# tnwei/waternet

Hardware: NVIDIA H100
Metric: images/sec at 1080p batch16 (preprocess + gated-fusion forward, uint8 in -> uint8 out) (higher is better)
Workload: dtype bf16 + fp8 corrections (v = hi + lo: hi x hi in bf16, both correction terms of the heavy layers as one e4m3 MMA; fp32 accumulate; 3-term bf16 elsewhere)

## Files before the change

### waternet_b200/csrc/conv_umma.cu

```cuda
#include "umma_conv.cuh"

namespace wn {

__device__ __forceinline__ bool pack_pixel(const PackInArgs& a, int n, int y, int x, float* v) {
  bool exact = true;
#pragma unroll
  for (int t = 0; t < 4; t++)
#pragma unroll
    for (int c = 0; c < 3; c++) {
      float f = __fmul_rn(a.p[t][n * a.s[t][0] + c * a.s[t][1] + y * a.s[t][2] + x * a.s[t][3]], 255.0f);
      float r = rintf(f);
      if (fabsf(f - r) <= 6.103515625e-5f && r >= 0.f && r <= 255.f) f = r; else exact = false;
      v[t * 3 + c] = f;
    }
  return exact;
}
template <bool HI>
__device__ __forceinline__ void store_packed(uint4* o, int hw, float* v) {
  v[12] = v[13] = v[14] = v[15] = 0.f;
  uint32_t hi[8], lo[8];
#pragma unroll
  for (int j = 0; j < 16; j += 2) {
    if constexpr (HI) {
      const __nv_bfloat162 hb = __floats2bfloat162_rn(v[j], v[j + 1]);
      hi[j >> 1] = *reinterpret_cast<const uint32_t*>(&hb);
      lo[j >> 1] = 0u;
    } else {
      split_bf16x2(v[j], v[j + 1], hi[j >> 1], lo[j >> 1]);
    }
  }
  o[0] = make_uint4(hi[0], hi[1], hi[2], hi[3]);
  o[hw] = make_uint4(hi[4], hi[5], hi[6], hi[7]);
  o[2 * (size_t)hw] = make_uint4(lo[0], lo[1], lo[2], lo[3]);
  o[3 * (size_t)hw] = make_uint4(lo[4], lo[5], lo[6], lo[7]);
}
__device__ __forceinline__ bool pack_slot_pixel(const PackInArgs& a, const SlotPixel& p, float* v) {
  return pack_pixel(a, p.img, p.y, p.x, v);
}
__device__ __forceinline__ bool pack_slot_pixel(const PackInArgs* __restrict__ imgs, const SlotPixel& p, float* v) {
  return pack_pixel(imgs[p.img], 0, p.y, p.x, v);
}

template <class Geom, class In, bool PLANES, bool FLAG, bool HI = false>
__global__ void __launch_bounds__(256)
pack_inputs_kernel(Geom geo, In in, uint4* __restrict__ out, int* __restrict__ exact_flag) {
  const int pix = blockIdx.x * 256 + threadIdx.x;
  const int hw = geo.slot_hw();
  bool exact = true;
  if (pix < hw) {
    const SlotPixel p = geo.at(blockIdx.y, pix);
    float v[16];
#pragma unroll
    for (int j = 0; j < 12; j++) v[j] = 0.f;
    if (p.valid) exact = pack_slot_pixel(in, p, v);
    if constexpr (PLANES) store_packed<HI>(out + (size_t)blockIdx.y * 4 * hw + pix, hw, v);
  }
  if constexpr (FLAG)
    if (!__syncthreads_and(exact) && threadIdx.x == 0) atomicExch(exact_flag, 0);
}

template <bool PLANES, bool FLAG, class Geom, class In>
static int launch_pack(wn_handle* h, const Geom& geo, const In& in, int count, uint4* act0, int* flag, bool reset,
                       cudaStream_t stream, bool hi = false) {
  TimedScope ts(h, kSlotPack, stream);
  if (reset) WN_CUDA(cudaMemsetAsync(flag, 1, sizeof(int), stream));
  const dim3 grid((unsigned)(((size_t)geo.slot_hw() + 255) / 256), count);
  if (PLANES && hi)
    pack_inputs_kernel<Geom, In, PLANES, FLAG, true><<<grid, 256, 0, stream>>>(geo, in, act0, flag);
  else
    pack_inputs_kernel<Geom, In, PLANES, FLAG><<<grid, 256, 0, stream>>>(geo, in, act0, flag);
  WN_LAUNCH_CHECK(h);
  return WN_OK;
}
int pack_inputs(wn_handle* h, const GridGeom& geo, const PackInArgs& in, int count, uint4* act0, int* flag,
                cudaStream_t stream, bool hi) {
  if (!act0) return launch_pack<false, true>(h, geo, in, count, nullptr, flag, true, stream);
  if (flag) return launch_pack<true, true>(h, geo, in, count, act0, flag, true, stream, hi);
  return launch_pack<true, false>(h, geo, in, count, act0, nullptr, false, stream, hi);
}
int pack_inputs(wn_handle* h, const TableGeom& geo, const PackInArgs* imgs, int count, uint4* act0, int* flag,
                cudaStream_t stream, bool hi) {
  if (!act0) return launch_pack<false, true>(h, geo, imgs, count, nullptr, flag, false, stream);
  return launch_pack<true, false>(h, geo, imgs, count, act0, nullptr, false, stream, hi);
}

__global__ void __launch_bounds__(256) store_kept_kernel(const float* __restrict__ src, int cs, int c0, int c,
                                                         float* __restrict__ dst, GridGeom geo) {
  const int pix = blockIdx.x * 256 + threadIdx.x;
  const int hw = geo.slot_hw();
  if (pix >= hw) return;
  const SlotPixel p = geo.at(blockIdx.y, pix);
  if (!p.kept) return;
  const float* s = src + ((size_t)blockIdx.y * cs + c0) * hw + pix;
  float* d = dst + (size_t)p.img * c * p.ihw + p.o;
  for (int k = 0; k < c; k++) d[k * p.ihw] = s[(size_t)k * hw];
}

enum UmmaLayer {
  kL1 = 0,
  kC2, kC3, kC4, kC5, kC6, kC7,
  kC8,
  kR2,
  kR3,
  kRL1,
  kNumUmmaLayers
};
struct UmmaLayerSpec {
  int ks, cinpad, npad, epi, concat, nblk, tps, slot;
  bool f8;
  int mw, ng, wgs;
};
static constexpr UmmaLayerSpec kSpecs[kNumUmmaLayers] = {
    {7, 16, 224, kEpiAct, 0, 1, 1, 0, false, 1, 1, 2},
    {5, 128, 128, kEpiAct, 0, 1, 5, 1, true, 1, 1, 2},
    {3, 128, 128, kEpiAct, 0, 1, 3, 2, true, 1, 1, 3},
    {1, 128, 64, kEpiAct, 1, 1, 1, 3, false, 1, 1, 3},
    {7, 64, 64, kEpiAct, 1, 1, 7, 4, true, 2, 1, 2},
    {5, 64, 64, kEpiAct, 1, 1, 5, 5, true, 2, 1, 2},
    {3, 64, 64, kEpiAct, 1, 1, 9, 6, true, 2, 1, 2},
    {3, 64, 16, kEpiSigmoid, 1, 1, 9, 7, false, 1, 1, 3},
    {5, 96, 32, kEpiAct, 1, 3, 5, 9, true, 1, 1, 3},
    {3, 96, 16, kEpiGate, 1, 1, 9, 10, false, 1, 1, 3},
    {7, 16, 96, kEpiAct, 0, 1, 1, 8, false, 1, 1, 3}};
#ifdef WN_UMMA_WGS2
static constexpr int layer_wgs(int) { return 2; }
#else
static constexpr int layer_wgs(int li) { return kSpecs[li].wgs; }
#endif

static_assert(kSpecs[kC2].f8 == kSpecs[kR2].f8, "L1 writes one format for both of its consumers");
static constexpr bool writes_f8(int li) { return li < kR3 && li != kC8 && kSpecs[li + 1].f8; }

static __global__ void __launch_bounds__(256)
mirror_u8_kernel(const uint8_t* __restrict__ src, PeerOut peers, size_t bytes, const int* __restrict__ run_if) {
  if (run_if && *run_if == 0) return;
  const size_t stride = (size_t)gridDim.x * blockDim.x, i0 = (size_t)blockIdx.x * blockDim.x + threadIdx.x;
#pragma unroll
  for (int k = 0; k < WN_MAX_PEERS; k++) {
    if (k >= peers.n) continue;
    uint8_t* dst = peers.p[k];
    const size_t vecs = (((reinterpret_cast<uintptr_t>(src) | reinterpret_cast<uintptr_t>(dst)) & 15) == 0) ? bytes / 16 : 0;
    for (size_t i = i0; i < vecs; i += stride) reinterpret_cast<uint4*>(dst)[i] = reinterpret_cast<const uint4*>(src)[i];
    for (size_t i = vecs * 16 + i0; i < bytes; i += stride) dst[i] = src[i];
  }
}
int mirror_u8(wn_handle* h, const uint8_t* src, const PeerOut& peers, size_t bytes, const int* run_if, cudaStream_t stream) {
  if (peers.n <= 0 || bytes == 0) return WN_OK;
  mirror_u8_kernel<<<4 * h->sm_count, 256, 0, stream>>>(src, peers, bytes, run_if);
  WN_LAUNCH_CHECK(h);
  return WN_OK;
}

struct UmmaWeights {
  uint8_t* stages8[kNumUmmaLayers];
  float* scale8[kNumUmmaLayers];
  int* overflow_dev;
  int* overflow_host;
  uint8_t* stages[kNumUmmaLayers];
  float* bias[kNumUmmaLayers];
  float* dense;
};

static size_t stage_bytes_total(const UmmaLayerSpec& s) { return (size_t)(s.cinpad / 16) * s.ks * s.ks * s.npad * 64; }

int umma_pack_weights(wn_handle* h, const float* const* params, cudaStream_t stream) {
  if (!h->umma) h->umma = (UmmaWeights*)calloc(1, sizeof(UmmaWeights));
  for (int i = 0; i < kNumUmmaLayers; i++) {
    if (!h->umma->stages[i]) WN_CUDA(cudaMalloc(&h->umma->stages[i], stage_bytes_total(kSpecs[i])));
    if (!h->umma->bias[i]) WN_CUDA(cudaMalloc(&h->umma->bias[i], kSpecs[i].npad * kSpecs[i].nblk * sizeof(float)));
    if (kSpecs[i].f8) {
      if (!h->umma->stages8[i]) WN_CUDA(cudaMalloc(&h->umma->stages8[i], stage_bytes_total(kSpecs[i])));
      if (!h->umma->scale8[i]) WN_CUDA(cudaMalloc(&h->umma->scale8[i], 4 * sizeof(float)));
    }
  }
  if (!h->umma->dense) WN_CUDA(cudaMalloc(&h->umma->dense, (size_t)224 * 128 * 49 * sizeof(float)));
  if (!h->umma->overflow_dev) WN_CUDA(cudaMalloc(&h->umma->overflow_dev, sizeof(int)));
  if (!h->umma->overflow_host) WN_CUDA(cudaHostAlloc(&h->umma->overflow_host, sizeof(int), cudaHostAllocDefault));
  UmmaWeights* u = h->umma;
  *u->overflow_host = 0;
  WN_CUDA(cudaMemsetAsync(u->overflow_dev, 0, sizeof(int), stream));
  auto W = [&](int conv) { return params[2 * conv]; };
  auto B = [&](int conv) { return params[2 * conv + 1]; };
  for (int li = 0; li < kNumUmmaLayers; li++) {
    const UmmaLayerSpec& s = kSpecs[li];
    const int kk = s.ks * s.ks;
    const int rows = s.npad * s.nblk;
    WN_CUDA(cudaMemsetAsync(u->dense, 0, (size_t)rows * s.cinpad * kk * sizeof(float), stream));
    WN_CUDA(cudaMemsetAsync(u->bias[li], 0, rows * sizeof(float), stream));
    auto scatter = [&](int conv, int co, int ci, int row_off, int split, int base0, int base1) -> int {
      scatter_weights_kernel<<<128, 256, 0, stream>>>(W(conv), u->dense, co, ci, kk, s.cinpad, row_off, split,
                                                      base0, base1, li == kL1 || li == kRL1 ? 255.0f : 1.0f);
      WN_LAUNCH_CHECK(h);
      scatter_bias_kernel<<<1, 256, 0, stream>>>(B(conv), u->bias[li], co, row_off);
      WN_LAUNCH_CHECK(h);
      return WN_OK;
    };
    int rc = WN_OK;
    if (li == kL1) {
      rc = scatter(0, 128, 12, 0, 12, 0, 0);
      for (int r = 0; r < 3 && !rc; r++)
        rc = scatter(8 + 3 * r, 32, 6, 128 + 32 * r, 3, 0, 3 * (r + 1));
    } else if (li >= kC2 && li <= kC8) {
      const int conv = li;
      const LayerDesc& d = kCmg[conv];
      rc = scatter(conv, d.cout, d.cin, 0, d.cin, 0, 0);
    } else if (li == kR2) {
      for (int r = 0; r < 3 && !rc; r++) rc = scatter(8 + 3 * r + 1, 32, 32, 32 * r, 32, 32 * r, 0);
    } else if (li == kRL1) {
      for (int r = 0; r < 3 && !rc; r++) rc = scatter(8 + 3 * r, 32, 6, 32 * r, 3, 0, 3 * (r + 1));
    } else {
      for (int r = 0; r < 3 && !rc; r++) rc = scatter(8 + 3 * r + 2, 3, 32, 3 * r, 32, 32 * r, 0);
    }
    if (rc) return rc;
    const int gw = s.npad / s.ng;
    const size_t group_bytes = stage_bytes_total(s) / s.ng;
    for (int g = 0; g < s.ng; g++) {
      pack_stages_kernel<<<256, 256, 0, stream>>>(u->dense, (__nv_bfloat16*)(u->stages[li] + g * group_bytes), gw,
                                                  s.cinpad, kk, s.concat, s.nblk, g * gw);
      WN_LAUNCH_CHECK(h);
    }
    if (s.f8) {
      WN_CUDA(cudaMemsetAsync(u->scale8[li], 0, 4 * sizeof(float), stream));
      f8_absmax_kernel<<<64, 256, 0, stream>>>(u->dense, (size_t)rows * s.cinpad * kk, u->scale8[li]);
      WN_LAUNCH_CHECK(h);
      f8_scale_finish_kernel<<<1, 1, 0, stream>>>(u->scale8[li]);
      WN_LAUNCH_CHECK(h);
      for (int g = 0; g < s.ng; g++) {
        pack_stages_f8_kernel<<<256, 256, 0, stream>>>(u->dense, u->stages8[li] + g * group_bytes, u->scale8[li], gw,
                                                       s.cinpad, kk, s.nblk, g * gw);
        WN_LAUNCH_CHECK(h);
      }
    }
  }
  return WN_OK;
}

void umma_free(wn_handle* h) {
  if (!h->umma) return;
  for (int i = 0; i < kNumUmmaLayers; i++) {
    if (h->umma->stages[i]) cudaFree(h->umma->stages[i]);
    if (h->umma->bias[i]) cudaFree(h->umma->bias[i]);
    if (h->umma->stages8[i]) cudaFree(h->umma->stages8[i]);
    if (h->umma->scale8[i]) cudaFree(h->umma->scale8[i]);
  }
  if (h->umma->dense) cudaFree(h->umma->dense);
  if (h->umma->overflow_dev) cudaFree(h->umma->overflow_dev);
  if (h->umma->overflow_host) cudaFreeHost(h->umma->overflow_host);
  free(h->umma);
  h->umma = nullptr;
}

static constexpr size_t kUmmaBytesPerPixel = 64 + 512 + 512 + 384 + 384 + 12;

static constexpr long long kDefaultChunkPixels = 8ll << 20;
static int umma_chunk(long long cap, int n, int h, int w) {
  if (cap <= 0 || cap > kDefaultChunkPixels) cap = kDefaultChunkPixels;
  long long per = (long long)h * w;
  long long nb = cap / (per > 0 ? per : 1);
  if (nb < 1) nb = 1;
  return nb < n ? (int)nb : n;
}
int umma_chunk_images(const wn_handle* h, int n, int height, int width) {
  return umma_chunk(h ? h->chunk_pixels : 0, n, height, width);
}

size_t umma_forward_workspace_bytes(int n, int h, int w) {
  const size_t nb = (size_t)umma_chunk(0, n, h, w);
  return nb * h * w * kUmmaBytesPerPixel + nb * h * 64 + 4096;
}

// ... 579 lines not shown
```

### waternet_b200/csrc/umma_conv.cuh

```cuda
#pragma once

#include <cuda.h>
#include <cuda_bf16.h>

#include "common.cuh"
#include "wgmma_ops.cuh"

namespace wn {

__device__ __forceinline__ uint32_t smem_u32(const void* p) {
  return (uint32_t)__cvta_generic_to_shared(p);
}
__device__ __forceinline__ void mbar_init(uint64_t* bar, uint32_t count) {
  asm volatile("mbarrier.init.shared::cta.b64 [%0], %1;" ::"r"(smem_u32(bar)), "r"(count));
}
__device__ __forceinline__ void mbar_wait(uint64_t* bar, uint32_t parity) {
  for (uint32_t it = 0; it < (1u << 26); it++) {
    uint32_t done;
    asm volatile(
        "{\n\t.reg .pred p;\n\t"
        "mbarrier.try_wait.parity.shared::cta.b64 p, [%1], %2;\n\t"
        "selp.u32 %0, 1, 0, p;\n\t}"
        : "=r"(done)
        : "r"(smem_u32(bar)), "r"(parity)
        : "memory");
    if (done) return;
  }
  __trap();
}
__device__ __forceinline__ void mbar_arrive(uint64_t* bar) {
  asm volatile("mbarrier.arrive.shared::cta.b64 _, [%0];" ::"r"(smem_u32(bar)) : "memory");
}
__device__ __forceinline__ void mbar_expect_tx(uint64_t* bar, uint32_t bytes) {
  asm volatile("mbarrier.arrive.expect_tx.shared::cta.b64 _, [%0], %1;" ::"r"(smem_u32(bar)), "r"(bytes)
               : "memory");
}
__device__ __forceinline__ void tma_load_5d(void* dst, const CUtensorMap* tmap, uint64_t* bar, int c0,
                                            int c1, int c2, int c3, int c4) {
  asm volatile(
      "cp.async.bulk.tensor.5d.shared::cluster.global.mbarrier::complete_tx::bytes [%0], [%1, {%3, %4, %5, %6, %7}], [%2];"
      ::"r"(smem_u32(dst)), "l"(tmap), "r"(smem_u32(bar)), "r"(c0), "r"(c1), "r"(c2), "r"(c3), "r"(c4)
      : "memory");
}
__device__ __forceinline__ void bulk_load(void* dst, const void* src, uint32_t bytes, uint64_t* bar) {
  asm volatile(
      "cp.async.bulk.shared::cluster.global.mbarrier::complete_tx::bytes [%0], [%1], %2, [%3];" ::"r"(
          smem_u32(dst)),
      "l"(src), "r"(bytes), "r"(smem_u32(bar))
      : "memory");
}
__device__ __forceinline__ uint64_t make_desc(uint32_t addr, uint32_t lbo, uint32_t sbo) {
  return (uint64_t)((addr >> 4) & 0x3fff) | ((uint64_t)((lbo >> 4) & 0x3fff) << 16) |
         ((uint64_t)((sbo >> 4) & 0x3fff) << 32);
}
__device__ __forceinline__ void wg_fence() { asm volatile("wgmma.fence.sync.aligned;" ::: "memory"); }
__device__ __forceinline__ void wg_commit() { asm volatile("wgmma.commit_group.sync.aligned;" ::: "memory"); }
template <int PENDING>
__device__ __forceinline__ void wg_wait() { asm volatile("wgmma.wait_group.sync.aligned %0;" ::"n"(PENDING) : "memory"); }
__device__ __forceinline__ void wg_bar(int id) { asm volatile("bar.sync %0, 128;" ::"r"(id) : "memory"); }
__device__ __forceinline__ uint32_t pack_e4m3x4(float f0, float f1, float f2, float f3) {
  uint16_t lo, hi;
  asm("cvt.rn.satfinite.e4m3x2.f32 %0, %1, %2;" : "=h"(lo) : "f"(f1), "f"(f0));
  asm("cvt.rn.satfinite.e4m3x2.f32 %0, %1, %2;" : "=h"(hi) : "f"(f3), "f"(f2));
  return (uint32_t)lo | ((uint32_t)hi << 16);
}
__device__ __forceinline__ uint16_t pack_e4m3x2(float f0, float f1) {
  uint16_t v;
  asm("cvt.rn.satfinite.e4m3x2.f32 %0, %1, %2;" : "=h"(v) : "f"(f1), "f"(f0));
  return v;
}

enum Epilogue { kEpiAct = 0, kEpiSigmoid = 1, kEpiGate = 2, kEpiDgrad = 3 };

constexpr int kStageLd = 36;

constexpr int kFmtIn8 = 1, kFmtOut8 = 2, kFmtHi = 4;
constexpr int kWgs3ProducerRegs = 24, kWgs3ConsumerRegs = 160;
template <int KS, int CIN_PAD, int NPAD, int CONCAT = 0, int NBLK = 1, int TPS = 1, int FMT = 0, int MW = 1,
          int NG = 1, int WGS = 2>
struct UmmaCfg {
  static constexpr bool F8IN = (FMT & kFmtIn8) != 0;
  static constexpr bool HI = (FMT & kFmtHi) != 0;
  static constexpr bool DUAL = CONCAT != 0 && !HI;
  static constexpr int TILE_W = 8 * MW, TILE_H = 8 * WGS;
  static constexpr int CONSUMER_WARPS = 4 * WGS;
  static constexpr int WARP_A = CONSUMER_WARPS, WARP_B = CONSUMER_WARPS + 1;
  static constexpr int THREADS = WGS == 2 ? 320 : 512;
  static constexpr int HALO_W = TILE_W + KS - 1, HALO_H = TILE_H + KS - 1;
  static constexpr int NCHUNK = CIN_PAD / 16;
  static constexpr int PLANE_BYTES = HALO_W * HALO_H * 16;
  static constexpr int A_STAGE = (4 * PLANE_BYTES + 1023) / 1024 * 1024;
  static constexpr int B_TAP = NPAD * 64;
  static constexpr int B_STAGE = TPS * B_TAP;
  static_assert((KS * KS) % TPS == 0, "taps per weight stage must divide the filter");
  static constexpr int NSTAGE_PER_CHUNK = KS * KS / TPS;
  static constexpr int STAGING = WGS * 64 * kStageLd * 4;
  static constexpr int BIAS_BYTES = NG * NBLK * NPAD * 4;
  static constexpr int TAIL = 512 + (BIAS_BYTES > 1536 ? BIAS_BYTES : 1536);
  static constexpr int BUDGET = 227 * 1024 - 1024 - TAIL - STAGING;
  static constexpr int NA_WANT = NCHUNK == 1 ? 2 : KS == 1 ? 6 : 3;
  static constexpr int NB_FIT = (BUDGET - NA_WANT * A_STAGE) / B_STAGE;
  static constexpr int NB = NB_FIT > 8 ? 8 : NB_FIT < 2 ? 2 : NB_FIT;
  static constexpr int NA_FIT = (BUDGET - NB * B_STAGE) / A_STAGE;
  static constexpr int NA = NA_FIT > NA_WANT ? NA_WANT : NA_FIT;
  static_assert(!F8IN || !CONCAT, "fp8 corrections: the [hi | second part] weight layout");
  static_assert(!HI || FMT == kFmtHi, "single-pass bf16 reads and writes bf16 planes only");
  static constexpr int CPB = NCHUNK / NBLK;
  static constexpr int BLK_COLS = DUAL ? 2 * NPAD : NPAD;
  static constexpr int COLS = NBLK * BLK_COLS;
  static constexpr int ACC = COLS / 2;
  static constexpr int ACC8 = F8IN ? ACC : 1;
  static constexpr int SMEM_BYTES = NA * A_STAGE + NB * B_STAGE + STAGING + TAIL + 1024;
  static_assert(NA >= 1, "halo tile does not fit in shared memory");
  static_assert(NCHUNK % NBLK == 0, "chunks must split evenly over the diagonal blocks");
  static_assert(NPAD % 16 == 0 && (DUAL ? 2 : 1) * NPAD <= 256, "invalid wgmma N");
  static_assert(MW == 1 || MW == 2, "one or two m64 blocks per warpgroup");
  static_assert(WGS == 2 || (WGS == 3 && MW == 1), "two consumer warpgroups, or three of one m64 block each");
  static_assert(NG == 1 || NBLK == 1, "column groups of a block-diagonal layer");
  static_assert(MW * (ACC + (F8IN ? ACC8 : 0)) <= 128, "accumulators do not fit in registers");
  static constexpr size_t GROUP_BYTES = (size_t)NCHUNK * NSTAGE_PER_CHUNK * B_STAGE;
};

struct ActDst {
  uint4* base;
  int planes_half;
};

struct ConvArgs {
  const uint8_t* wpk;
  const float* bias;
  int N, H, W;
  int in_planes_half;
  int tiles_x, tiles_y;
  ActDst dst0, dst1;
  int split_c;
  int cout;
  float* out_f32;
  const float* cm;
  uint8_t* out_u8;
  const int* skip_lo;
  int a_hi_only;
  float* refined_out;
  const uint4* mask_base;
  int mask_planes_half;
  const float* f8_scale;
  int* f8_overflow;
  const int* run_if;
  int tiled;
  long long win0;
  TileGeom tiles;
  const RaggedWindow* rwin;
};

__device__ __forceinline__ uint32_t pack_bf16x2(__nv_bfloat16 a, __nv_bfloat16 b) {
  return (uint32_t)__bfloat16_as_ushort(a) | ((uint32_t)__bfloat16_as_ushort(b) << 16);
}
__device__ __forceinline__ void split_bf16x2(float f0, float f1, uint32_t& hi, uint32_t& lo) {
  const __nv_bfloat162 h = __floats2bfloat162_rn(f0, f1);
  hi = *reinterpret_cast<const uint32_t*>(&h);
  const float h0 = __uint_as_float(hi << 16), h1 = __uint_as_float(hi & 0xffff0000u);
  const __nv_bfloat162 l = __floats2bfloat162_rn(f0 - h0, f1 - h1);
  lo = *reinterpret_cast<const uint32_t*>(&l);
}

template <int EPI, bool OUT8, bool RAG = false, bool HI = false>
__device__ __forceinline__ void epilogue16(const ConvArgs& g, const float* s_bias, const float* f, int ch, int n,
                                           int gx, int gy, bool valid = true) {
  const size_t hw = (size_t)g.H * g.W;
  const size_t pix = (size_t)gy * g.W + gx;
  if constexpr (EPI == kEpiAct || EPI == kEpiDgrad) {
    if (ch >= g.cout) return;
    if constexpr (OUT8) {
      uint32_t hi[8], l8[4], h8[4];
      float vmax = 0.f;
#pragma unroll
      for (int j = 0; j < 16; j += 4) {
        float v[4], r[4];
#pragma unroll
        for (int t = 0; t < 4; t++) {
          v[t] = fmaxf(f[j + t] + s_bias[ch + j + t], 0.f);
          if constexpr (RAG) v[t] = valid ? v[t] : 0.f;
          vmax = fmaxf(vmax, v[t]);
        }
#pragma unroll
        for (int t = 0; t < 4; t += 2) {
          const __nv_bfloat162 h = __floats2bfloat162_rn(v[t], v[t + 1]);
          const uint32_t hb = *reinterpret_cast<const uint32_t*>(&h);
          hi[(j + t) >> 1] = hb;
          r[t] = (v[t] - __uint_as_float(hb << 16)) * 512.f;
          r[t + 1] = (v[t + 1] - __uint_as_float(hb & 0xffff0000u)) * 512.f;
        }
        l8[j >> 2] = pack_e4m3x4(r[0], r[1], r[2], r[3]);
        h8[j >> 2] = pack_e4m3x4(v[0], v[1], v[2], v[3]);
      }
      if (!(vmax <= 448.f) && g.f8_overflow) atomicOr(g.f8_overflow, 1);
      const bool second = ch >= g.split_c;
      const ActDst& d = second ? g.dst1 : g.dst0;
      const int chl = second ? ch - g.split_c : ch;
      uint4* p_hi = d.base + ((size_t)n * 2 * d.planes_half + (chl >> 3)) * hw + pix;
      uint4* p_f8 = d.base + ((size_t)n * 2 * d.planes_half + d.planes_half + 2 * (chl >> 4)) * hw + pix;
      p_hi[0] = make_uint4(hi[0], hi[1], hi[2], hi[3]);
      p_hi[hw] = make_uint4(hi[4], hi[5], hi[6], hi[7]);
      p_f8[0] = make_uint4(l8[0], l8[1], l8[2], l8[3]);
      p_f8[hw] = make_uint4(h8[0], h8[1], h8[2], h8[3]);
    } else {
#pragma unroll
      for (int q = 0; q < 16; q += 8) {
        const int c = ch + q;
        if (c >= g.cout) break;
        uint32_t hi[4], lo[4];
        uint32_t mask[4] = {0xffffffffu, 0xffffffffu, 0xffffffffu, 0xffffffffu};
        if constexpr (EPI == kEpiDgrad) {
          if (g.mask_base) {
            const uint4 m = g.mask_base[((size_t)n * 2 * g.mask_planes_half + (c >> 3)) * hw + pix];
            mask[0] = m.x; mask[1] = m.y; mask[2] = m.z; mask[3] = m.w;
          }
        }
#pragma unroll
        for (int j = 0; j < 8; j += 2) {
          float f0, f1;
          if constexpr (EPI == kEpiDgrad) {
            f0 = (mask[j >> 1] & 0x0000ffffu) ? f[q + j] : 0.f;
            f1 = (mask[j >> 1] & 0xffff0000u) ? f[q + j + 1] : 0.f;
          } else {
            f0 = fmaxf(f[q + j] + s_bias[c + j], 0.f);
            f1 = fmaxf(f[q + j + 1] + s_bias[c + j + 1], 0.f);
            if constexpr (RAG) {
              f0 = valid ? f0 : 0.f;
              f1 = valid ? f1 : 0.f;
            }
          }
          if constexpr (HI) {
            const __nv_bfloat162 hb = __floats2bfloat162_rn(f0, f1);
            hi[j >> 1] = *reinterpret_cast<const uint32_t*>(&hb);
            lo[j >> 1] = 0u;
          } else {
            split_bf16x2(f0, f1, hi[j >> 1], lo[j >> 1]);
          }
        }
        const bool second = c >= g.split_c;
        const ActDst& d = second ? g.dst1 : g.dst0;
        const int plane = (second ? c - g.split_c : c) >> 3;
        uint4* p_hi = d.base + ((size_t)n * 2 * d.planes_half + plane) * hw + pix;
        p_hi[0] = make_uint4(hi[0], hi[1], hi[2], hi[3]);
        p_hi[(size_t)d.planes_half * hw] = make_uint4(lo[0], lo[1], lo[2], lo[3]);
      }
    }
  } else {
    if (ch != 0) return;
    const size_t o = (size_t)n * 3 * hw + pix;
    if constexpr (EPI == kEpiSigmoid) {
#pragma unroll
      for (int c = 0; c < 3; c++) g.out_f32[o + c * hw] = 1.0f / (1.0f + expf(-(f[c] + s_bias[c])));
    } else {
      float r[9];
#pragma unroll
      for (int j = 0; j < 9; j++) r[j] = fmaxf(f[j] + s_bias[j], 0.f);
      if (g.refined_out) {
#pragma unroll
        for (int j = 0; j < 9; j++) g.refined_out[(size_t)n * 9 * hw + pix + j * hw] = r[j];
      }
      if (g.cm) {
        const float c0 = g.cm[o], c1 = g.cm[o + hw], c2 = g.cm[o + 2 * hw];
        float v[3];
#pragma unroll
        for (int c = 0; c < 3; c++)
          v[c] = __fadd_rn(__fadd_rn(__fmul_rn(r[c], c0), __fmul_rn(r[3 + c], c1)), __fmul_rn(r[6 + c], c2));
        size_t oo = o, ohw = hw, o8 = ((size_t)n * hw + pix) * 3;
        float* out_f32 = g.out_f32;
        uint8_t* out_u8 = g.out_u8;
        if constexpr (RAG) {
          const RaggedWindow& t = g.rwin[n];
          const int y = t.ys + gy, x = t.xs + gx;
          if (y < t.ky0 || y >= t.ky1 || x < t.kx0 || x >= t.kx1) return;
          ohw = (size_t)t.H * t.W;
          oo = (size_t)y * t.W + x;
          o8 = oo * 3;
          out_f32 = t.out_f32;
          out_u8 = t.out_u8;
        } else if (g.tiled) {
          const TileWindow t = tile_window(g.tiles, g.win0 + n);
          const int y = t.ys + gy, x = t.xs + gx;
          if (y < t.ky0 || y >= t.ky1 || x < t.kx0 || x >= t.kx1) return;
          ohw = (size_t)g.tiles.H * g.tiles.W;
          const size_t ipix = (size_t)y * g.tiles.W + x;
          oo = (size_t)t.img * 3 * ohw + ipix;
          o8 = ((size_t)t.img * ohw + ipix) * 3;
        }
        if (out_f32) {
#pragma unroll
          for (int c = 0; c < 3; c++) out_f32[oo + c * ohw] = v[c];
        }
        if (out_u8) {
          uint8_t* q = out_u8 + o8;
#pragma unroll
          for (int c = 0; c < 3; c++) q[c] = (uint8_t)(int)__fmul_rn(fminf(fmaxf(v[c], 0.0f), 1.0f), 255.0f);
        }
      }
    }
  }
}

template <int KS, int CIN_PAD, int NPAD, int EPI, int CONCAT, int NBLK, int TPS, int FMT = 0, bool RAG = false,
          int MW = 1, int NG = 1, int WGS = 2>
__global__ void __launch_bounds__(WGS == 2 ? 320 : 512, 1)
conv_umma_kernel(const __grid_constant__ CUtensorMap tmap_in, const ConvArgs g) {
  using C = UmmaCfg<KS, CIN_PAD, NPAD, CONCAT, NBLK, TPS, FMT, MW, NG, WGS>;
  constexpr bool F8IN = C::F8IN, DUAL = C::DUAL, OUT8 = (FMT & kFmtOut8) != 0;
  static_assert(!OUT8 || EPI == kEpiAct, "fp8 planes are written by the activation epilogue only");
  static_assert(!RAG || EPI == kEpiAct || EPI == kEpiGate, "ragged passes mask activations and store the gate");
  if (g.run_if != nullptr && *reinterpret_cast<const volatile int*>(g.run_if) == 0) return;
  extern __shared__ uint8_t smem_raw[];
  uint8_t* smem = reinterpret_cast<uint8_t*>((reinterpret_cast<uintptr_t>(smem_raw) + 1023) & ~(uintptr_t)1023);
  uint8_t* a_stages = smem;
  uint8_t* b_stages = smem + C::NA * C::A_STAGE;
  float* staging = reinterpret_cast<float*>(b_stages + C::NB * C::B_STAGE);
  uint8_t* tail = reinterpret_cast<uint8_t*>(staging) + C::STAGING;
  uint64_t* a_full = reinterpret_cast<uint64_t*>(tail);
  uint64_t* a_empty = a_full + C::NA;
  uint64_t* b_full = a_empty + C::NA;
  uint64_t* b_empty = b_full + C::NB;
  float* s_bias = reinterpret_cast<float*>(tail + 512);
  static_assert((2 * 6 + 2 * 8) * 8 <= 512 && C::BIAS_BYTES <= C::TAIL - 512, "barrier / bias area");

  const int tid = threadIdx.x, warp = tid >> 5, lane = tid & 31;
  const int num_tiles = g.tiles_x * g.tiles_y * g.N * NG;
  if (tid == 0) {
    for (int i = 0; i < C::NA; i++) { mbar_init(&a_full[i], 1); mbar_init(&a_empty[i], C::CONSUMER_WARPS); }
    for (int i = 0; i < C::NB; i++) { mbar_init(&b_full[i], 1); mbar_init(&b_empty[i], C::CONSUMER_WARPS); }
    asm volatile("fence.mbarrier_init.release.cluster;" ::: "memory");
  }
  for (int i = tid; i < NG * NBLK * NPAD; i += C::THREADS) s_bias[i] = g.bias[i];
  __syncthreads();
  if constexpr (WGS == 3) {
    if (warp >= C::CONSUMER_WARPS) {
      asm volatile("setmaxnreg.dec.sync.aligned.u32 %0;" ::"n"(kWgs3ProducerRegs));
      if (warp > C::WARP_B) return;
    }
  }
  if (warp == C::WARP_A) {
    if (lane == 0) {
      int stage = 0;
      uint32_t phase = 0;
      for (int tile = blockIdx.x; tile < num_tiles; tile += gridDim.x) {
        const int pt = tile / NG;
        const int n = pt / (g.tiles_x * g.tiles_y);
        const int rem = pt - n * g.tiles_x * g.tiles_y;
        const int ty = rem / g.tiles_x, tx = rem - ty * g.tiles_x;
        const int x0 = tx * C::TILE_W - KS / 2, y0 = ty * C::TILE_H - KS / 2;
        for (int c = 0; c < C::NCHUNK; c++) {
          mbar_wait(&a_empty[stage], phase ^ 1);
          uint8_t* dst = a_stages + stage * C::A_STAGE;
          mbar_expect_tx(&a_full[stage], (C::HI || g.a_hi_only ? 2 : 4) * C::PLANE_BYTES);
          tma_load_5d(dst, &tmap_in, &a_full[stage], 0, x0, y0, 2 * c, n);
          if (!C::HI && !g.a_hi_only)
            tma_load_5d(dst + 2 * C::PLANE_BYTES, &tmap_in, &a_full[stage], 0, x0, y0, g.in_planes_half + 2 * c, n);
          if (++stage == C::NA) { stage = 0; phase ^= 1; }
        }
      }
    }
    return;
  }
  if (warp == C::WARP_B) {
    if (lane == 0) {
      int stage = 0;
      uint32_t phase = 0;
      for (int tile = blockIdx.x; tile < num_tiles; tile += gridDim.x) {
        const uint8_t* wpk = g.wpk + (size_t)(tile % NG) * C::GROUP_BYTES;
        for (int it = 0; it < C::NCHUNK * C::NSTAGE_PER_CHUNK; it++) {
          mbar_wait(&b_empty[stage], phase ^ 1);
          mbar_expect_tx(&b_full[stage], C::B_STAGE);
          bulk_load(b_stages + stage * C::B_STAGE, wpk + (size_t)it * C::B_STAGE, C::B_STAGE, &b_full[stage]);
          if (++stage == C::NB) { stage = 0; phase ^= 1; }
        }
      }
    }
    return;
  }
  if constexpr (WGS == 3) asm volatile("setmaxnreg.inc.sync.aligned.u32 %0;" ::"n"(kWgs3ConsumerRegs));

  const int wg = warp >> 2, wtid = tid & 127;
  const bool skip_lo = (g.skip_lo != nullptr && *g.skip_lo != 0) || g.a_hi_only;
  const float dscale0 = F8IN && WGS == 2 ? *g.f8_scale : 1.f;
  constexpr uint32_t kSboA = C::HALO_W * 16;
  constexpr uint32_t kLboB = (CONCAT ? 2 * NPAD : NPAD) * 16;
  float acc[MW][C::ACC], acc8[MW][C::ACC8];
  int astage = 0, bstage = 0, pend_a = -1, pend_b = -1;
  uint32_t aphase = 0, bphase = 0;
  auto release = [&]() {
    if (lane == 0) {
      if (pend_b >= 0) mbar_arrive(&b_empty[pend_b]);
      if (pend_a >= 0) mbar_arrive(&a_empty[pend_a]);
    }
    pend_a = pend_b = -1;
  };
  for (int tile = blockIdx.x; tile < num_tiles; tile += gridDim.x) {
#pragma unroll
    for (int mb = 0; mb < MW; mb++) {
#pragma unroll
      for (int i = 0; i < C::ACC; i++) acc[mb][i] = 0.f;
#pragma unroll
      for (int i = 0; i < C::ACC8; i++) acc8[mb][i] = 0.f;
    }
#pragma unroll
    for (int c = 0; c < C::NCHUNK; c++) {
      mbar_wait(&a_full[astage], aphase);
      const uint32_t a_base = smem_u32(a_stages + astage * C::A_STAGE) + (uint32_t)(wg * 8 * C::HALO_W * 16);
      const int blk = NBLK > 1 ? c / C::CPB : 0;
      for (int tg = 0; tg < C::NSTAGE_PER_CHUNK; tg++) {
        mbar_wait(&b_full[bstage], bphase);
        const uint32_t b_base = smem_u32(b_stages + bstage * C::B_STAGE);
        wg_fence();
#pragma unroll
        for (int t = 0; t < TPS; t++) {
          const int tap = tg * TPS + t;
          const int ky = tap / KS, kx = tap - ky * KS;
          const uint32_t a_tap = a_base + (uint32_t)((ky * C::HALO_W + kx) * 16);
          const uint32_t b_tap = b_base + (uint32_t)(t * C::B_TAP);
          const uint64_t a_hi0 = make_desc(a_tap, C::PLANE_BYTES, kSboA);
#pragma unroll
          for (int mb = 0; mb < MW; mb++) {
            const uint64_t a_hi = a_hi0 + mb * (128 >> 4);
            const uint64_t a_lo = MW == 1 ? make_desc(a_tap + 2 * C::PLANE_BYTES, C::PLANE_BYTES, kSboA)
                                          : a_hi + ((2 * C::PLANE_BYTES) >> 4);
#pragma unroll
            for (int b = 0; b < NBLK; b++) {
              if (NBLK > 1 && b != blk) continue;
              float* d = acc[mb] + b * C::BLK_COLS / 2;
              if constexpr (C::HI) {
                wgmma_bf16<NPAD>(d, a_hi, make_desc(b_tap, kLboB, 128));
              } else if constexpr (F8IN) {
                wgmma_bf16<NPAD>(d, a_hi, make_desc(b_tap, NPAD * 16, 128));
                wgmma_e4m3<NPAD>(acc8[mb] + b * C::BLK_COLS / 2, a_lo, make_desc(b_tap + NPAD * 32, NPAD * 16, 128));
              } else if constexpr (CONCAT) {
                wgmma_bf16<2 * NPAD>(d, a_hi, make_desc(b_tap, kLboB, 128));
                if (!skip_lo) wgmma_bf16<NPAD>(d, a_lo, make_desc(b_tap, kLboB, 128));
              } else {
                wgmma_bf16<NPAD>(d, a_hi, make_desc(b_tap, kLboB, 128));
                if (!skip_lo) wgmma_bf16<NPAD>(d, a_lo, make_desc(b_tap, kLboB, 128));
                wgmma_bf16<NPAD>(d, a_hi, make_desc(b_tap + 2 * NPAD * 16, kLboB, 128));
              }
            }
          }
        }
        wg_commit();
        wg_wait<1>();
        release();
        pend_b = bstage;
        if (tg == C::NSTAGE_PER_CHUNK - 1) pend_a = astage;
        if (++bstage == C::NB) { bstage = 0; bphase ^= 1; }
      }
      if (++astage == C::NA) { astage = 0; aphase ^= 1; }
    }
    wg_wait<0>();
    release();

    const int pt = tile / NG, c0 = (tile % NG) * NPAD;
    const int n = pt / (g.tiles_x * g.tiles_y);
    const int rem = pt - n * g.tiles_x * g.tiles_y;
    const int ty = rem / g.tiles_x, tx = rem - ty * g.tiles_x;
    float* stg = staging + wg * 64 * kStageLd;
    const int frow = (warp & 3) * 16 + (lane >> 2), fcol = (lane & 3) * 2;
    const int r = wtid & 63, half = wtid >> 6;
    const int m = wg * 64 + r;
    const int gy = ty * C::TILE_H + (m >> 3);
    const float dscale = F8IN && WGS == 3 ? *g.f8_scale : dscale0;
    constexpr int NCH = NBLK * NPAD;
#pragma unroll
    for (int mb = 0; mb < MW; mb++) {
      const int gx = tx * C::TILE_W + mb * 8 + (m & 7);
      const bool inside = gx < g.W && gy < g.H;
      bool valid = true;
      if constexpr (RAG) valid = gx < g.rwin[n].vw && gy < g.rwin[n].vh;
#pragma unroll
      for (int ch0 = 0; ch0 < NCH; ch0 += 32) {
#pragma unroll
        for (int j = 0; j < 4; j++) {
          const int ch = ch0 + 8 * j;
          if (ch < NCH) {
            const int col = NBLK > 1 ? (ch / NPAD) * C::BLK_COLS + ch % NPAD : ch;
            float v[4];
#pragma unroll
            for (int k = 0; k < 4; k++) {
              v[k] = acc[mb][col / 2 + k];
              if constexpr (DUAL) v[k] += acc[mb][(col + NPAD) / 2 + k];
              if constexpr (F8IN) v[k] = (v[k] + acc8[mb][col / 2 + k]) * dscale;
            }
            float* s = stg + frow * kStageLd + 8 * j + fcol;
            *reinterpret_cast<float2*>(s) = make_float2(v[0], v[1]);
            *reinterpret_cast<float2*>(s + 8 * kStageLd) = make_float2(v[2], v[3]);
          }
        }
        wg_bar(1 + wg);
        const int cb = ch0 + 16 * half;
        if (cb < NCH && inside) {
          float f[16];
          const float4* s = reinterpret_cast<const float4*>(stg + r * kStageLd + 16 * half);
#pragma unroll
          for (int q = 0; q < 4; q++) {
            const float4 x = s[q];
            f[4 * q] = x.x; f[4 * q + 1] = x.y; f[4 * q + 2] = x.z; f[4 * q + 3] = x.w;
          }
          epilogue16<EPI, OUT8, RAG, C::HI>(g, s_bias, f, c0 + cb, n, gx, gy, valid);
        }
        wg_bar(1 + wg);
      }
    }
  }
}

static __global__ void scatter_weights_kernel(const float* __restrict__ src, float* __restrict__ dense, int co, int ci,
                                       int kk, int cinpad, int row_off, int split, int base0, int base1,
                                       float divisor) {
  const int total = co * ci * kk;
  for (int i = blockIdx.x * blockDim.x + threadIdx.x; i < total; i += gridDim.x * blockDim.x) {
    int t = i % kk;
    int c = (i / kk) % ci;
    int o = i / (kk * ci);
    int cd = c < split ? base0 + c : base1 + (c - split);
    dense[((size_t)(row_off + o) * cinpad + cd) * kk + t] = __fdiv_rn(src[i], divisor);
  }
}
static __global__ void scatter_bias_kernel(const float* __restrict__ src, float* __restrict__ dst, int co, int row_off) {
  for (int i = blockIdx.x * blockDim.x + threadIdx.x; i < co; i += gridDim.x * blockDim.x) dst[row_off + i] = src[i];
}
static __global__ void pack_stages_kernel(const float* __restrict__ dense, __nv_bfloat16* __restrict__ out, int npad,
                                   int cinpad, int kk, int concat, int nblk, int row_off = 0) {
  const int nchunk = cinpad / 16, cpb = nchunk / nblk;
  const size_t total = (size_t)nchunk * kk * 2 * 2 * npad * 8;
  for (size_t i = (size_t)blockIdx.x * blockDim.x + threadIdx.x; i < total; i += (size_t)gridDim.x * blockDim.x) {
    int e = (int)(i % 8);
    size_t r = i / 8;
    int k8, split, nrow;
    if (concat) {
      int row2 = (int)(r % (2 * npad)); r /= 2 * npad;
      k8 = (int)(r % 2); r /= 2;
      split = row2 >= npad;
      nrow = row2 - split * npad;
    } else {
      nrow = (int)(r % npad); r /= npad;
      k8 = (int)(r % 2); r /= 2;
      split = (int)(r % 2); r /= 2;
    }
    int tap = (int)(r % kk);
    int chunk = (int)(r / kk);
    int cin = chunk * 16 + k8 * 8 + e;
    int row = row_off + (chunk / cpb) * npad + nrow;
    float w = dense[((size_t)row * cinpad + cin) * kk + tap];
    __nv_bfloat16 hi = __float2bfloat16_rn(w);
    out[i] = split == 0 ? hi : __float2bfloat16_rn(w - __bfloat162float(hi));
  }
}


static __global__ void f8_absmax_kernel(const float* __restrict__ dense, size_t n, float* __restrict__ scale) {
  __shared__ float smax[256];
  float m = 0.f;
  for (size_t i = (size_t)blockIdx.x * blockDim.x + threadIdx.x; i < n; i += (size_t)gridDim.x * blockDim.x)
    m = fmaxf(m, fabsf(dense[i]));
  smax[threadIdx.x] = m;
  __syncthreads();
  for (int o = 128; o > 0; o >>= 1) {
    if ((int)threadIdx.x < o) smax[threadIdx.x] = fmaxf(smax[threadIdx.x], smax[threadIdx.x + o]);
    __syncthreads();
  }
  if (threadIdx.x == 0) atomicMax(reinterpret_cast<unsigned int*>(scale + 2), __float_as_uint(smax[0]));
}
static __global__ void f8_scale_finish_kernel(float* __restrict__ scale) {
  const float mx = fmaxf(scale[2], 1e-30f);
  const float ws = exp2f(floorf(log2f(224.f / mx)));
  scale[0] = ws;
  scale[1] = 1.f / (512.f * ws);
}
static __global__ void pack_stages_f8_kernel(const float* __restrict__ dense, uint8_t* __restrict__ out,
                                             const float* __restrict__ scale, int npad, int cinpad, int kk, int nblk,
                                             int row_off) {
  const int nchunk = cinpad / 16, cpb = nchunk / nblk, rows = npad;
  const size_t tap_bytes = (size_t)rows * 64;
  const float ws = scale[0];
  const size_t total = (size_t)nchunk * kk * rows * 8;
  for (size_t i = (size_t)blockIdx.x * blockDim.x + threadIdx.x; i < total; i += (size_t)gridDim.x * blockDim.x) {
    size_t r = i;
    const int cp = (int)(r % 8); r /= 8;
    const int row = (int)(r % rows); r /= rows;
    const int tap = (int)(r % kk);
    const int chunk = (int)(r / kk);
    const int wrow = row_off + (chunk / cpb) * npad + row;
    float w[2], wl[2];
    uint16_t hb[2];
#pragma unroll
    for (int t = 0; t < 2; t++) {
      w[t] = dense[((size_t)wrow * cinpad + chunk * 16 + 2 * cp + t) * kk + tap];
      const __nv_bfloat16 h = __float2bfloat16_rn(w[t]);
      hb[t] = __bfloat16_as_ushort(h);
      wl[t] = w[t] - __bfloat162float(h);
    }
    uint8_t* base = out + ((size_t)chunk * kk + tap) * tap_bytes;
    const int c = 2 * cp;
#pragma unroll
    for (int t = 0; t < 2; t++)
      hb[t] = __bfloat16_as_ushort(__float2bfloat16_rn(__bfloat162float(__ushort_as_bfloat16(hb[t])) * ws * 512.f));
    *reinterpret_cast<uint32_t*>(base + ((size_t)(c / 8) * rows + row) * 16 + (c % 8) * 2) =
        (uint32_t)hb[0] | ((uint32_t)hb[1] << 16);
    uint8_t* p1 = base + (size_t)rows * 32;
    *reinterpret_cast<uint16_t*>(p1 + ((size_t)0 * rows + row) * 16 + c) = pack_e4m3x2(w[0] * ws, w[1] * ws);
// ... 66 lines not shown
```

Baseline: 54.09.

## Let consumer warps issue their own TMA refills for three-warpgroup two-block conv

Adds a SELF_LOAD mode for WGS=3, MW=2 layers in which the dedicated producer warps are removed. Consumers refill stages themselves: after arriving on an empty barrier, a warp checks with test_wait whether the stage is fully freed and claims the refill with a shared-memory atomic max. Stage and phase are derived from monotonically increasing counters, and the block drops to 384 threads with no setmaxnreg split. The 7x7 64-channel layer is switched to three warpgroups to use this path. The aim is a larger M tile (24 rows by 16 columns) with fewer threads and no producer warps. The cost is refill latency now sitting on the consumer path, and possibly fewer A stages.

```diff
diff --git a/waternet_b200/csrc/conv_umma.cu b/waternet_b200/csrc/conv_umma.cu
--- a/waternet_b200/csrc/conv_umma.cu
+++ b/waternet_b200/csrc/conv_umma.cu
@@ -115,7 +115,7 @@
     {5, 128, 128, kEpiAct, 0, 1, 5, 1, true, 1, 1, 2},
     {3, 128, 128, kEpiAct, 0, 1, 3, 2, true, 1, 1, 3},
     {1, 128, 64, kEpiAct, 1, 1, 1, 3, false, 1, 1, 3},
-    {7, 64, 64, kEpiAct, 1, 1, 7, 4, true, 2, 1, 2},
+    {7, 64, 64, kEpiAct, 1, 1, 7, 4, true, 2, 1, 3},
     {5, 64, 64, kEpiAct, 1, 1, 5, 5, true, 2, 1, 2},
     {3, 64, 64, kEpiAct, 1, 1, 9, 6, true, 2, 1, 2},
     {3, 64, 16, kEpiSigmoid, 1, 1, 9, 7, false, 1, 1, 3},
diff --git a/waternet_b200/csrc/umma_conv.cuh b/waternet_b200/csrc/umma_conv.cuh
--- a/waternet_b200/csrc/umma_conv.cuh
+++ b/waternet_b200/csrc/umma_conv.cuh
@@ -31,6 +31,22 @@
 __device__ __forceinline__ void mbar_arrive(uint64_t* bar) {
   asm volatile("mbarrier.arrive.shared::cta.b64 _, [%0];" ::"r"(smem_u32(bar)) : "memory");
 }
+__device__ __forceinline__ bool mbar_test(uint64_t* bar, uint32_t parity) {
+  uint32_t done;
+  asm volatile(
+      "{\n\t.reg .pred p;\n\t"
+      "mbarrier.test_wait.parity.shared::cta.b64 p, [%1], %2;\n\t"
+      "selp.u32 %0, 1, 0, p;\n\t}"
+      : "=r"(done)
+      : "r"(smem_u32(bar)), "r"(parity)
+      : "memory");
+  return done != 0;
+}
+__device__ __forceinline__ int smem_max(int* p, int v) {
+  int old;
+  asm volatile("atom.relaxed.cta.shared::cta.max.s32 %0, [%1], %2;" : "=r"(old) : "r"(smem_u32(p)), "r"(v) : "memory");
+  return old;
+}
 __device__ __forceinline__ void mbar_expect_tx(uint64_t* bar, uint32_t bytes) {
   asm volatile("mbarrier.arrive.expect_tx.shared::cta.b64 _, [%0], %1;" ::"r"(smem_u32(bar)), "r"(bytes)
                : "memory");
@@ -85,7 +101,8 @@
   static constexpr int TILE_W = 8 * MW, TILE_H = 8 * WGS;
   static constexpr int CONSUMER_WARPS = 4 * WGS;
   static constexpr int WARP_A = CONSUMER_WARPS, WARP_B = CONSUMER_WARPS + 1;
-  static constexpr int THREADS = WGS == 2 ? 320 : 512;
+  static constexpr bool SELF_LOAD = WGS == 3 && MW == 2;
+  static constexpr int THREADS = WGS == 2 ? 320 : SELF_LOAD ? 384 : 512;
   static constexpr int HALO_W = TILE_W + KS - 1, HALO_H = TILE_H + KS - 1;
   static constexpr int NCHUNK = CIN_PAD / 16;
   static constexpr int PLANE_BYTES = HALO_W * HALO_H * 16;
@@ -98,7 +115,9 @@
   static constexpr int BIAS_BYTES = NG * NBLK * NPAD * 4;
   static constexpr int TAIL = 512 + (BIAS_BYTES > 1536 ? BIAS_BYTES : 1536);
   static constexpr int BUDGET = 227 * 1024 - 1024 - TAIL - STAGING;
-  static constexpr int NA_WANT = NCHUNK == 1 ? 2 : KS == 1 ? 6 : 3;
+  static constexpr int NA_WANT0 = NCHUNK == 1 ? 2 : KS == 1 ? 6 : 3;
+  static constexpr int NA_WANT =
+      SELF_LOAD && NA_WANT0 == 3 && (BUDGET - 3 * A_STAGE) / B_STAGE < 3 ? 2 : NA_WANT0;
   static constexpr int NB_FIT = (BUDGET - NA_WANT * A_STAGE) / B_STAGE;
   static constexpr int NB = NB_FIT > 8 ? 8 : NB_FIT < 2 ? 2 : NB_FIT;
   static constexpr int NA_FIT = (BUDGET - NB * B_STAGE) / A_STAGE;
@@ -115,7 +134,7 @@
   static_assert(NCHUNK % NBLK == 0, "chunks must split evenly over the diagonal blocks");
   static_assert(NPAD % 16 == 0 && (DUAL ? 2 : 1) * NPAD <= 256, "invalid wgmma N");
   static_assert(MW == 1 || MW == 2, "one or two m64 blocks per warpgroup");
-  static_assert(WGS == 2 || (WGS == 3 && MW == 1), "two consumer warpgroups, or three of one m64 block each");
+  static_assert(WGS == 2 || WGS == 3, "two or three consumer warpgroups");
   static_assert(NG == 1 || NBLK == 1, "column groups of a block-diagonal layer");
   static_assert(MW * (ACC + (F8IN ? ACC8 : 0)) <= 128, "accumulators do not fit in registers");
   static constexpr size_t GROUP_BYTES = (size_t)NCHUNK * NSTAGE_PER_CHUNK * B_STAGE;
@@ -301,9 +320,48 @@
   }
 }
 
+template <class C, int KS, int NG>
+__device__ __forceinline__ void fill_a(const CUtensorMap* tmap, const ConvArgs& g, uint8_t* a_stages,
+                                       uint64_t* a_full, int k) {
+  const int tile = blockIdx.x + (k / C::NCHUNK) * gridDim.x, c = k % C::NCHUNK, stage = k % C::NA;
+  const int pt = tile / NG;
+  const int n = pt / (g.tiles_x * g.tiles_y);
+  const int rem = pt - n * g.tiles_x * g.tiles_y;
+  const int ty = rem / g.tiles_x, tx = rem - ty * g.tiles_x;
+  const int x0 = tx * C::TILE_W - KS / 2, y0 = ty * C::TILE_H - KS / 2;
+  uint8_t* dst = a_stages + stage * C::A_STAGE;
+  mbar_expect_tx(&a_full[stage], (C::HI || g.a_hi_only ? 2 : 4) * C::PLANE_BYTES);
+  tma_load_5d(dst, tmap, &a_full[stage], 0, x0, y0, 2 * c, n);
+  if (!C::HI && !g.a_hi_only)
+    tma_load_5d(dst + 2 * C::PLANE_BYTES, tmap, &a_full[stage], 0, x0, y0, g.in_planes_half + 2 * c, n);
+}
+template <class C, int NG>
+__device__ __forceinline__ void fill_b(const ConvArgs& g, uint8_t* b_stages, uint64_t* b_full, int k) {
+  constexpr int PER_TILE = C::NCHUNK * C::NSTAGE_PER_CHUNK;
+  const int tile = blockIdx.x + (k / PER_TILE) * gridDim.x, it = k % PER_TILE, stage = k % C::NB;
+  const uint8_t* wpk = g.wpk + (size_t)(tile % NG) * C::GROUP_BYTES;
+  mbar_expect_tx(&b_full[stage], C::B_STAGE);
+  bulk_load(b_stages + stage * C::B_STAGE, wpk + (size_t)it * C::B_STAGE, C::B_STAGE, &b_full[stage]);
+}
+template <int NSTAGE, int PER>
+__device__ __forceinline__ bool stage_freed_by_last(int* issued, uint64_t* empty, int k, int num_tiles) {
+  const int s = k % NSTAGE;
+  if (!mbar_test(&empty[s], (uint32_t)(k / NSTAGE) & 1)) return false;
+  if (smem_max(&issued[s], k + NSTAGE + 1) >= k + NSTAGE + 1) return false;
+  return (int)blockIdx.x + (k + NSTAGE) / PER * (int)gridDim.x < num_tiles;
+}
+template <bool SELF_LOAD, int NSTAGE>
+__device__ __forceinline__ int ring_stage(int s) {
+  if constexpr (SELF_LOAD) return s % NSTAGE; else return s;
+}
+template <bool SELF_LOAD, int NSTAGE>
+__device__ __forceinline__ uint32_t ring_phase(int s, uint32_t phase) {
+  if constexpr (SELF_LOAD) return (uint32_t)(s / NSTAGE) & 1; else return phase;
+}
+
 template <int KS, int CIN_PAD, int NPAD, int EPI, int CONCAT, int NBLK, int TPS, int FMT = 0, bool RAG = false,
           int MW = 1, int NG = 1, int WGS = 2>
-__global__ void __launch_bounds__(WGS == 2 ? 320 : 512, 1)
+__global__ void __launch_bounds__(WGS == 2 ? 320 : MW == 2 ? 384 : 512, 1)
 conv_umma_kernel(const __grid_constant__ CUtensorMap tmap_in, const ConvArgs g) {
   using C = UmmaCfg<KS, CIN_PAD, NPAD, CONCAT, NBLK, TPS, FMT, MW, NG, WGS>;
   constexpr bool F8IN = C::F8IN, DUAL = C::DUAL, OUT8 = (FMT & kFmtOut8) != 0;
@@ -321,63 +379,76 @@
   uint64_t* b_full = a_empty + C::NA;
   uint64_t* b_empty = b_full + C::NB;
   float* s_bias = reinterpret_cast<float*>(tail + 512);
-  static_assert((2 * 6 + 2 * 8) * 8 <= 512 && C::BIAS_BYTES <= C::TAIL - 512, "barrier / bias area");
+  static_assert((2 * 6 + 2 * 8) * 8 <= 256 && 256 + (6 + 8) * 4 <= 512 && C::BIAS_BYTES <= C::TAIL - 512,
+                "barrier / counter / bias area");
 
   const int tid = threadIdx.x, warp = tid >> 5, lane = tid & 31;
   const int num_tiles = g.tiles_x * g.tiles_y * g.N * NG;
   if (tid == 0) {
     for (int i = 0; i < C::NA; i++) { mbar_init(&a_full[i], 1); mbar_init(&a_empty[i], C::CONSUMER_WARPS); }
     for (int i = 0; i < C::NB; i++) { mbar_init(&b_full[i], 1); mbar_init(&b_empty[i], C::CONSUMER_WARPS); }
+    if constexpr (C::SELF_LOAD)
+      for (int i = 0; i < C::NA + C::NB; i++) reinterpret_cast<int*>(tail + 256)[i] = 0;
     asm volatile("fence.mbarrier_init.release.cluster;" ::: "memory");
   }
   for (int i = tid; i < NG * NBLK * NPAD; i += C::THREADS) s_bias[i] = g.bias[i];
   __syncthreads();
-  if constexpr (WGS == 3) {
-    if (warp >= C::CONSUMER_WARPS) {
-      asm volatile("setmaxnreg.dec.sync.aligned.u32 %0;" ::"n"(kWgs3ProducerRegs));
-      if (warp > C::WARP_B) return;
-    }
-  }
-  if (warp == C::WARP_A) {
-    if (lane == 0) {
-      int stage = 0;
-      uint32_t phase = 0;
-      for (int tile = blockIdx.x; tile < num_tiles; tile += gridDim.x) {
-        const int pt = tile / NG;
-        const int n = pt / (g.tiles_x * g.tiles_y);
-        const int rem = pt - n * g.tiles_x * g.tiles_y;
-        const int ty = rem / g.tiles_x, tx = rem - ty * g.tiles_x;
-        const int x0 = tx * C::TILE_W - KS / 2, y0 = ty * C::TILE_H - KS / 2;
-        for (int c = 0; c < C::NCHUNK; c++) {
-          mbar_wait(&a_empty[stage], phase ^ 1);
-          uint8_t* dst = a_stages + stage * C::A_STAGE;
-          mbar_expect_tx(&a_full[stage], (C::HI || g.a_hi_only ? 2 : 4) * C::PLANE_BYTES);
-          tma_load_5d(dst, &tmap_in, &a_full[stage], 0, x0, y0, 2 * c, n);
-          if (!C::HI && !g.a_hi_only)
-            tma_load_5d(dst + 2 * C::PLANE_BYTES, &tmap_in, &a_full[stage], 0, x0, y0, g.in_planes_half + 2 * c, n);
-          if (++stage == C::NA) { stage = 0; phase ^= 1; }
-        }
-      }
-    }
-    return;
-  }
-  if (warp == C::WARP_B) {
-    if (lane == 0) {
-      int stage = 0;
-      uint32_t phase = 0;
-      for (int tile = blockIdx.x; tile < num_tiles; tile += gridDim.x) {
-        const uint8_t* wpk = g.wpk + (size_t)(tile % NG) * C::GROUP_BYTES;
-        for (int it = 0; it < C::NCHUNK * C::NSTAGE_PER_CHUNK; it++) {
-          mbar_wait(&b_empty[stage], phase ^ 1);
-          mbar_expect_tx(&b_full[stage], C::B_STAGE);
-          bulk_load(b_stages + stage * C::B_STAGE, wpk + (size_t)it * C::B_STAGE, C::B_STAGE, &b_full[stage]);
-          if (++stage == C::NB) { stage = 0; phase ^= 1; }
-        }
-      }
-    }
-    return;
-  }
-  if constexpr (WGS == 3) asm volatile("setmaxnreg.inc.sync.aligned.u32 %0;" ::"n"(kWgs3ConsumerRegs));
+  if constexpr (C::SELF_LOAD) {
+    if (tid == 0) {
+      const int total_a = (num_tiles - (int)blockIdx.x + (int)gridDim.x - 1) / (int)gridDim.x * C::NCHUNK;
+      const int total_b = total_a * C::NSTAGE_PER_CHUNK;
+      for (int k = 0; k < C::NA && k < total_a; k++) fill_a<C, KS, NG>(&tmap_in, g, a_stages, a_full, k);
+      for (int k = 0; k < C::NB && k < total_b; k++) fill_b<C, NG>(g, b_stages, b_full, k);
+    }
+  }
+  if constexpr (!C::SELF_LOAD) {
+    if constexpr (WGS == 3) {
+      if (warp >= C::CONSUMER_WARPS) {
+        asm volatile("setmaxnreg.dec.sync.aligned.u32 %0;" ::"n"(kWgs3ProducerRegs));
+        if (warp > C::WARP_B) return;
+      }
+    }
+    if (warp == C::WARP_A) {
+      if (lane == 0) {
+        int stage = 0;
+        uint32_t phase = 0;
+        for (int tile = blockIdx.x; tile < num_tiles; tile += gridDim.x) {
+          const int pt = tile / NG;
+          const int n = pt / (g.tiles_x * g.tiles_y);
+          const int rem = pt - n * g.tiles_x * g.tiles_y;
+          const int ty = rem / g.tiles_x, tx = rem - ty * g.tiles_x;
+          const int x0 = tx * C::TILE_W - KS / 2, y0 = ty * C::TILE_H - KS / 2;
+          for (int c = 0; c < C::NCHUNK; c++) {
+            mbar_wait(&a_empty[stage], phase ^ 1);
+            uint8_t* dst = a_stages + stage * C::A_STAGE;
+            mbar_expect_tx(&a_full[stage], (C::HI || g.a_hi_only ? 2 : 4) * C::PLANE_BYTES);
+            tma_load_5d(dst, &tmap_in, &a_full[stage], 0, x0, y0, 2 * c, n);
+            if (!C::HI && !g.a_hi_only)
+              tma_load_5d(dst + 2 * C::PLANE_BYTES, &tmap_in, &a_full[stage], 0, x0, y0, g.in_planes_half + 2 * c, n);
+            if (++stage == C::NA) { stage = 0; phase ^= 1; }
+          }
+        }
+      }
+      return;
+    }
+    if (warp == C::WARP_B) {
+      if (lane == 0) {
+        int stage = 0;
+        uint32_t phase = 0;
+        for (int tile = blockIdx.x; tile < num_tiles; tile += gridDim.x) {
+          const uint8_t* wpk = g.wpk + (size_t)(tile % NG) * C::GROUP_BYTES;
+          for (int it = 0; it < C::NCHUNK * C::NSTAGE_PER_CHUNK; it++) {
+            mbar_wait(&b_empty[stage], phase ^ 1);
+            mbar_expect_tx(&b_full[stage], C::B_STAGE);
+            bulk_load(b_stages + stage * C::B_STAGE, wpk + (size_t)it * C::B_STAGE, C::B_STAGE, &b_full[stage]);
+            if (++stage == C::NB) { stage = 0; phase ^= 1; }
+          }
+        }
+      }
+      return;
+    }
+    if constexpr (WGS == 3) asm volatile("setmaxnreg.inc.sync.aligned.u32 %0;" ::"n"(kWgs3ConsumerRegs));
+  }
 
   const int wg = warp >> 2, wtid = tid & 127;
   const bool skip_lo = (g.skip_lo != nullptr && *g.skip_lo != 0) || g.a_hi_only;
@@ -389,8 +460,19 @@
   uint32_t aphase = 0, bphase = 0;
   auto release = [&]() {
     if (lane == 0) {
-      if (pend_b >= 0) mbar_arrive(&b_empty[pend_b]);
-      if (pend_a >= 0) mbar_arrive(&a_empty[pend_a]);
+      if (pend_b >= 0) {
+        mbar_arrive(&b_empty[ring_stage<C::SELF_LOAD, C::NB>(pend_b)]);
+        if constexpr (C::SELF_LOAD)
+          if (stage_freed_by_last<C::NB, C::NCHUNK * C::NSTAGE_PER_CHUNK>(reinterpret_cast<int*>(tail + 256) + C::NA,
+                                                                         b_empty, pend_b, num_tiles))
+            fill_b<C, NG>(g, b_stages, b_full, pend_b + C::NB);
+      }
+      if (pend_a >= 0) {
+        mbar_arrive(&a_empty[ring_stage<C::SELF_LOAD, C::NA>(pend_a)]);
+        if constexpr (C::SELF_LOAD)
+          if (stage_freed_by_last<C::NA, C::NCHUNK>(reinterpret_cast<int*>(tail + 256), a_empty, pend_a, num_tiles))
+            fill_a<C, KS, NG>(&tmap_in, g, a_stages, a_full, pend_a + C::NA);
+      }
     }
     pend_a = pend_b = -1;
   };
@@ -404,12 +486,13 @@
     }
 #pragma unroll
     for (int c = 0; c < C::NCHUNK; c++) {
-      mbar_wait(&a_full[astage], aphase);
-      const uint32_t a_base = smem_u32(a_stages + astage * C::A_STAGE) + (uint32_t)(wg * 8 * C::HALO_W * 16);
+      mbar_wait(&a_full[ring_stage<C::SELF_LOAD, C::NA>(astage)], ring_phase<C::SELF_LOAD, C::NA>(astage, aphase));
+      const uint32_t a_base =
+          smem_u32(a_stages + ring_stage<C::SELF_LOAD, C::NA>(astage) * C::A_STAGE) + (uint32_t)(wg * 8 * C::HALO_W * 16);
       const int blk = NBLK > 1 ? c / C::CPB : 0;
       for (int tg = 0; tg < C::NSTAGE_PER_CHUNK; tg++) {
-        mbar_wait(&b_full[bstage], bphase);
-        const uint32_t b_base = smem_u32(b_stages + bstage * C::B_STAGE);
+        mbar_wait(&b_full[ring_stage<C::SELF_LOAD, C::NB>(bstage)], ring_phase<C::SELF_LOAD, C::NB>(bstage, bphase));
+        const uint32_t b_base = smem_u32(b_stages + ring_stage<C::SELF_LOAD, C::NB>(bstage) * C::B_STAGE);
         wg_fence();
 #pragma unroll
         for (int t = 0; t < TPS; t++) {
@@ -448,9 +531,11 @@
         release();
         pend_b = bstage;
         if (tg == C::NSTAGE_PER_CHUNK - 1) pend_a = astage;
-        if (++bstage == C::NB) { bstage = 0; bphase ^= 1; }
-      }
-      if (++astage == C::NA) { astage = 0; aphase ^= 1; }
+        if constexpr (C::SELF_LOAD) bstage++;
+        else if (++bstage == C::NB) { bstage = 0; bphase ^= 1; }
+      }
+      if constexpr (C::SELF_LOAD) astage++;
+      else if (++astage == C::NA) { astage = 0; aphase ^= 1; }
     }
     wg_wait<0>();
     release();
```

Result: faster. 54.95 (median of 6 runs) (+1.6%).
